# Frikallo/parakeet.cpp

Measured on NVIDIA H100. Metric: audio-seconds/sec (RTFx) tdt-ctc-110m 10s clips, higher is better.
Workload: dtype bf16x3

## Files before the change

parakeet.cpp_b200/csrc/engine.cu:

```cuda
#include "engine.h"

#include <algorithm>
#include <cstdlib>
#include <unordered_map>

namespace pk_detail {
std::string &create_err() {
    thread_local std::string s;
    return s;
}
}
#define g_create_err (create_err())


pk_status pk_engine::get_vec(const SafeTensors &st, const std::string &name, int n, float **out) {
    std::vector<float> h;
    std::string e;
    if (!st.read_f32(name, h, n, e)) return fail(PK_ERR_MISSING, e);
    *out = upload(h);
    return *out ? PK_OK : fail(PK_ERR_CUDA, "cudaMalloc failed for " + name);
}

pk_status pk_engine::finish_weight(std::vector<float> &w, std::vector<float> *b, int N, int K, GemmWeight &out) {
    out.N = N;
// ... 312 lines not shown
    logmel = dalloc<float>(B * (size_t)Fmax * c.mel_bins);
    mel_part = dalloc<float>(mel_part_floats((int)B, c.mel_bins));
    feats = dalloc<float>(B * (size_t)Fmax * c.mel_bins);
    sub1 = act_alloc(rows2, C);
    sub2 = dalloc<float>(rows2 * C);
    sub3 = act_alloc(rows3, C);
    sub4 = act_alloc(rows3, C);
    if (cfg.math != PK_MATH_FP32 && sub4.hi && (!make_tc_operand(&sub4.tc, sub4.hi, sub4.lo, Mx, (size_t)C * f3n, 128) || !make_tc_operand(&sub4.tc32, sub4.hi, sub4.lo, Mx, (size_t)C * f3n, 32))) sub4.hi = nullptr;
    x = dalloc<float>(Mx * d);
    ln = act_alloc(Mx, d);
    ffh = act_alloc(Mx, c.ff);
    qkv = dalloc<float>(Mx * 3 * d);
    if (cfg.math != PK_MATH_FP32 && (c.d_model / c.n_heads == 64 || c.d_model / c.n_heads == 128)) {
        qkvp_hi = dalloc<bf16>(Mx * 2 * d);
        qkvp_lo = dalloc<bf16>(Mx * 2 * d);
        if (!qkvp_hi || !qkvp_lo) return fail(PK_ERR_CUDA, "cudaMalloc failed (qkv planes)");
    }
    ctx = act_alloc(Mx, d);
    glu = dalloc<float>(Mx * d);
    cv = act_alloc(Mx, d);
    const int ldv = (c.vocab + 3) & ~3;
    logits = dalloc<float>(Mx * ldv);
    EP = dalloc<float>(Mx * c.joint_hidden);
    best = dalloc<int32_t>(Mx);
    bconf = dalloc<float>(Mx);
    tok = dalloc<int32_t>(B * (1 + (size_t)cap));
    t_start = dalloc<int32_t>(B * (size_t)cap);
    t_end = dalloc<int32_t>(B * (size_t)cap);
    t_conf = dalloc<float>(B * (size_t)cap);
    Bpad = ((Bmax + 31) / 32) * 32;
    const size_t HS = (size_t)c.pred_hidden * Bpad;
    hbuf = dalloc<float>(HS * 2 * c.lstm_layers);
    zbuf = dalloc<float>((size_t)c.joint_hidden * Bpad);
    tdt_ints = dalloc<int32_t>((size_t)Bpad + 512);
    tdt_keys = dalloc<unsigned long long>((size_t)6 * Bpad + 8);
    const size_t PG = (size_t)3 * num_sms * Bpad;
    pl_max = dalloc<float>(PG);
    pl_sum = dalloc<float>(PG);
    skinny_ws_floats = (size_t)2 << 20;
    skinny_ws = dalloc<float>(skinny_ws_floats);
    skinny_tickets = dalloc<unsigned int>(SKINNY_TICKETS);
    if (skinny_tickets) cudaMemsetAsync(skinny_tickets, 0, SKINNY_TICKETS * sizeof(unsigned int), stream);
    if (!pl_sum || !tdt_keys || !hbuf || !x || !sub2 || !d_pcm || !t_conf || !skinny_ws || !skinny_tickets || !mel_part) return fail(PK_ERR_CUDA, "cudaMalloc failed (workspace)");
    if (cfg.math != PK_MATH_FP32 && (!sub1.hi || !sub3.hi || !sub4.hi || !ln.hi || !ffh.hi || !ctx.hi || !cv.hi))
        return fail(PK_ERR_CUDA, "workspace: cudaMalloc or cuTensorMapEncodeTiled failed for an activation operand");
    if (diar) {
        const int Dt = sf.t_hidden;
        t_x = dalloc<float>(Mx * Dt);
        t_qkv = dalloc<float>(Mx * 3 * Dt);
        if (cfg.math != PK_MATH_FP32) {
            t_kv_hi = dalloc<bf16>(Mx * 2 * Dt);
            if (cfg.math == PK_MATH_BF16X3) t_kv_lo = dalloc<bf16>(Mx * 2 * Dt);
            if (!t_kv_hi || (cfg.math == PK_MATH_BF16X3 && !t_kv_lo)) return fail(PK_ERR_CUDA, "cudaMalloc failed (k | v planes)");
        }
        probs = dalloc<float>(Mx * sf.max_speakers);
        t_ln = act_alloc(Mx, Dt);
        t_ctx = act_alloc(Mx, Dt);
        t_ff = act_alloc(Mx, sf.t_ff);
        if (!t_x || !t_qkv || !probs || (cfg.math == PK_MATH_FP32 ? (!t_ln.f32 || !t_ctx.f32 || !t_ff.f32) : (!t_ln.hi || !t_ctx.hi || !t_ff.hi)))
            return fail(PK_ERR_CUDA, "cudaMalloc or cuTensorMapEncodeTiled failed (transformer workspace)");
        PK_CUDA(cudaMallocHost(&h_probs, Mx * sf.max_speakers * sizeof(float)));
    }
    PK_CUDA(cudaMallocHost(&h_pcm, (B * (size_t)c.max_samples + 8) * sizeof(float)));
    PK_CUDA(cudaMallocHost(&h_meta, (size_t)(8 * (B + 1)) * sizeof(int32_t)));
    PK_CUDA(cudaMallocHost(&h_tok, B * (1 + (size_t)cap) * sizeof(int32_t)));
    PK_CUDA(cudaMallocHost(&h_ts, B * (size_t)cap * sizeof(int32_t)));
    PK_CUDA(cudaMallocHost(&h_te, B * (size_t)cap * sizeof(int32_t)));
    PK_CUDA(cudaMallocHost(&h_tc, B * (size_t)cap * sizeof(float)));
    return PK_OK;
}

pk_status pk_engine::set_batch_shapes(const int32_t *n_frames, const int64_t *offsets, int n) {
    if (n <= 0) return fail(PK_ERR_INVALID, "empty batch");
    if (n > Bmax) return fail(PK_ERR_CAPACITY, "batch of " + std::to_string(n) + " exceeds max_batch " + std::to_string(Bmax));
    n_utt = n;
    probs_valid = false;
// ... 274 lines not shown
                launch_ctc_boosted_decode(logprobs_dev, best, bconf, d_row_off, n_utt, c.vocab, c.vocab - 1, cap, boost_trie(), tok, t_start, t_end, t_conf, stream);
            else
                launch_ctc_collapse(best, bconf, d_row_off, n_utt, c.vocab - 1, cap, tok, t_start, t_end, t_conf, stream);
        }
    }
    launches += greedy ? 2 : 3;
    last_tdt = false;
    PK_CUDA(cudaGetLastError());
    return PK_OK;
}

pk_status pk_engine::run_tdt() {
    TdtParams p{};
    p.Bpad = ((n_utt + 31) / 32) * 32; p.n_utt = n_utt; p.max_sym = cfg.max_symbols;
    p.max_steps = maxT + cap + 2; p.row_off = d_row_off; p.hbuf = hbuf;
    p.boost_on = boosting() ? 1 : 0; p.trie = boost_trie(); p.boost_bits = boost_bits; p.trie_active = trie_active; p.trie_nact = trie_nact;
    return tdt_decode(p);
}

pk_status pk_engine::tdt_decode(TdtParams &p) {
    const pk_config &c = cfg;
    EpiParams ep;
    ep.kind = EPI_BIAS_F32;
    ep.out_f32 = EP;
    ep.ldo = c.joint_hidden;
    gemm(enc_operand(this), c.d_model, enc_proj, M, ep);

    p.P = c.pred_hidden; p.J = c.joint_hidden; p.V = c.vocab; p.D = c.n_durations; p.L = c.lstm_layers;
    p.cap = cap; p.n_dur = c.n_durations;
    for (int i = 0; i < 8; ++i) p.durations[i] = c.durations[i];
    p.EP = EP; p.G0 = G0;
    for (int l = 0; l < c.lstm_layers; ++l) { p.Whh[l] = Whh_s[l]; p.Wih[l] = Wih_s[l]; p.bih[l] = bih[l]; }
    p.Wp = Wp_s; p.Wout = Wout_s; p.bout = bout;
    p.z = zbuf;
    p.overflow = tdt_ints; p.bar = reinterpret_cast<unsigned int *>(tdt_ints + Bpad);
    p.pl_max = pl_max; p.pl_sum = pl_sum;
    p.key_lab = tdt_keys; p.key_dur = tdt_keys + 3 * (size_t)Bpad;
    p.dbg = reinterpret_cast<long long *>(tdt_keys + 6 * (size_t)Bpad);
    p.tok = tok; p.t_start = t_start; p.t_end = t_end; p.t_conf = t_conf;
    if (!p.carry) PK_CUDA(cudaMemsetAsync(p.hbuf, 0, (size_t)p.P * p.Bpad * 2 * p.L * sizeof(float), stream));
    cudaError_t ce;
    {
        Scope sc(this, CAT_TDT);
        ce = launch_tdt_decode(p, num_sms, stream);
    }
    launches += 2;
    last_tdt = true;
    if (ce != cudaSuccess) return fail(PK_ERR_CUDA, std::string("tdt_decode launch: ") + cudaGetErrorString(ce));
    PK_CUDA(cudaGetLastError());
    return PK_OK;
}

pk_status pk_engine::run_diar_head() {
    const int Dt = sf.t_hidden, H = sf.t_heads;
    const bool f32 = cfg.math == PK_MATH_FP32;
    Act xo;
    if (f32) xo.f32 = t_x; else xo = t_ln;
    ActBuf planes;
    if (!f32) planes = t_ln;
    {
        EpiParams ep;
        ep.kind = EPI_BIAS_F32;
        ep.out_f32 = t_x;
        ep.ldo = Dt;
        gemm(enc_operand(this), cfg.d_model, t_proj, M, ep);
        if (!f32) {
            Scope sc(this, CAT_LAYERNORM);
// ... 1503 lines not shown
```

parakeet.cpp_b200/csrc/engine.h:

```cpp
#pragma once
#include <cuda_runtime.h>

#include <algorithm>
#include <cmath>
#include <cstdio>
#include <cstring>
#include <functional>
#include <map>
#include <memory>
#include <string>
#include <tuple>
#include <vector>

#include "../../include/parakeet_b200.h"
#include "kernels.h"
#include "nccl_dl.h"
#include "safetensors.h"

using namespace pk;


namespace pk_detail {

std::string &create_err();
// ... 142 lines not shown
    int cap = 0;

    MelTables mel_tb{};
    float *c1_w, *c1_b, *dw1_w, *dw1_b, *dw2_w, *dw2_b;
    float *dw2_wt = nullptr;
    GemmWeight conv2, conv3, proj;
    std::vector<LayerW> layers;
    GemmWeight ctc_head;
    GemmWeight enc_proj;
    float *G0 = nullptr;
    float *Whh[PK_MAX_LSTM] = {}, *Wih[PK_MAX_LSTM] = {}, *bih[PK_MAX_LSTM] = {};
    float *Whh_um[PK_MAX_LSTM] = {}, *Wih_um[PK_MAX_LSTM] = {};
    float *Wp = nullptr, *Wout = nullptr, *bout = nullptr;
    bf16 *Whh_s[PK_MAX_LSTM] = {}, *Wih_s[PK_MAX_LSTM] = {}, *Wp_s = nullptr, *Wout_s = nullptr;

    float *d_pcm = nullptr;
    float *d_pcm_alt = nullptr;
    cudaEvent_t ev_pcm_free[2] = {}, ev_prefetch = nullptr;
    int pcm_cur = 0;
    cudaEvent_t ev_join = nullptr;
    struct { const float *pcm = nullptr; int32_t n = 0; std::vector<int64_t> off; bool valid = false; } pref;
    int64_t *d_pcm_off = nullptr;
    int32_t *d_frame_off = nullptr, *d_s2_off = nullptr, *d_row_off = nullptr, *d_t2_rows = nullptr;
    float *logmel = nullptr, *feats = nullptr;
    float *mel_part = nullptr;
    Act sub1, sub3, sub4, ln, ffh, ctx, cv;
    float *sub2 = nullptr, *x = nullptr, *qkv = nullptr, *glu = nullptr, *logits = nullptr, *EP = nullptr;
    bf16 *qkvp_hi = nullptr, *qkvp_lo = nullptr;
    int32_t *best = nullptr;
    float *bconf = nullptr;
    int32_t *tok = nullptr, *t_start = nullptr, *t_end = nullptr;
    float *t_conf = nullptr;
    int Bpad = 0;
    float *hbuf = nullptr, *cbuf = nullptr, *zbuf = nullptr, *pl_max = nullptr, *pl_sum = nullptr;
    int32_t *tdt_ints = nullptr;
    unsigned long long *tdt_keys = nullptr;
    float *h_pcm = nullptr;
    int32_t *h_meta = nullptr;
    int32_t *h_tok = nullptr, *h_ts = nullptr, *h_te = nullptr;
    float *h_tc = nullptr;

    struct GraphEntry { cudaGraphExec_t exec = nullptr; int64_t launches = 0; int seen = 0; };
    std::map<std::string, GraphEntry> graphs;
    bool use_graphs = true;
    bool attn_tc = true;

    int n_utt = 0;
    std::vector<int64_t> pcm_off;
    std::vector<int32_t> frame_off, s2_off, row_off, t2_rows;
    int maxF = 0, maxT2 = 0, maxT = 0, M = 0, M2 = 0;

    int32_t *job_tok = nullptr, *job_all = nullptr;
    int64_t job_cap_rows = 0, job_rows = 0, job_alloc_rows = 0;
    int job_world = 1;
    int32_t *h_job = nullptr;
    size_t h_job_ints = 0;
    float *job_pcm = nullptr;
    size_t job_pcm_cap = 0;
    std::vector<int64_t> job_off;
    const float *pcm_src = nullptr;
    float *d_raw = nullptr;
    size_t d_raw_cap = 0;
    int64_t *d_raw_off = nullptr;
    void *nccl_comm = nullptr;
    int nccl_rank = 0, nccl_world = 1;
    bool last_tdt = false;
    int32_t truncated = 0;
// ... 126 lines not shown
```

parakeet.cpp_b200/csrc/kernel_hooks.cu:

```cuda
#include <algorithm>
#include <cmath>
#include <cstring>
#include <vector>

#include "../../include/parakeet_b200.h"
#include "kernels.h"

using namespace pk;

namespace {

constexpr size_t kGuard = (size_t)64 << 10;

struct HookCtx {
    cudaStream_t st = nullptr;
    std::vector<void *> ptrs;
    struct Guarded {
        uint8_t *base;
        size_t bytes;
    };
    std::vector<Guarded> outs;
    bool ok = true;

    explicit HookCtx(int device) {
// ... 308 lines not shown
    auto split = [&](const float *w, int rows, int K) {
        float *dw = cx.upload(w, (size_t)rows * K);
        bf16 *s = static_cast<bf16 *>(cx.alloc((size_t)rows * 2 * K * sizeof(bf16)));
        if (s) launch_tdt_split_rows(dw, rows, K, s, cx.st);
        return static_cast<const bf16 *>(s);
    };
    std::vector<float> um((size_t)4 * P * P);
    for (int l = 0; l < L; ++l) {
        lstm_unit_major(in->W_hh[l], P, um.data());
        p.Whh[l] = split(um.data(), 4 * P, P);
        if (l > 0) {
            lstm_unit_major(in->W_ih[l], P, um.data());
            p.Wih[l] = split(um.data(), 4 * P, P);
            p.bih[l] = cx.upload(in->b_ih[l], (size_t)4 * P);
        }
    }
    p.Wp = split(in->W_p, J, P);
    p.Wout = split(in->W_out, NO, J);
    p.bout = cx.upload(in->b_out, NO);
    bf16 *hb = cx.guarded<bf16>(2 * L * 2 * HS);
    bf16 *zb = cx.guarded<bf16>((size_t)2 * Bpad * J);
    {
        std::vector<float> h((size_t)L * 2 * HS, 0.f);
        if (in->carry)
            for (int l = 0; l < L; ++l)
                for (int b = 0; b < n; ++b) memcpy(&h[(size_t)l * 2 * HS + (size_t)b * P], in->h0 + ((size_t)l * n + b) * P, (size_t)P * 4);
        float *dh = cx.upload(h.data(), h.size());
        if (!cx.ok) return PK_ERR_CUDA;
        ActBuf sh; sh.hi = hb; sh.lo = hb + (size_t)L * 2 * HS;
        launch_split(dh, h.size(), sh, cx.st);
    }
    p.hbuf = reinterpret_cast<float *>(hb);
    p.z = reinterpret_cast<float *>(zb);
    p.tok = cx.guarded<int32_t>((size_t)n * (1 + cap));
    p.t_start = cx.guarded<int32_t>((size_t)n * cap);
    p.t_end = cx.guarded<int32_t>((size_t)n * cap);
    p.t_conf = cx.guarded<float>((size_t)n * cap);
    p.overflow = cx.guarded<int32_t>(n);
    constexpr int kMaxGrid = 256;
    p.pl_max = static_cast<float *>(cx.alloc((size_t)3 * kMaxGrid * Bpad * sizeof(float)));
    p.pl_sum = static_cast<float *>(cx.alloc((size_t)3 * kMaxGrid * Bpad * sizeof(float)));
    p.key_lab = static_cast<unsigned long long *>(cx.alloc((size_t)3 * Bpad * 8));
    p.key_dur = static_cast<unsigned long long *>(cx.alloc((size_t)3 * Bpad * 8));
    p.bar = static_cast<unsigned int *>(cx.alloc(1024 * sizeof(unsigned int)));
    p.dbg = static_cast<long long *>(cx.alloc(8 * sizeof(long long)));
    if (in->carry) {
        p.carry = 1;
        std::vector<float> c((size_t)L * Bpad * P, 0.f);
        for (int l = 0; l < L; ++l)
            memcpy(&c[(size_t)l * Bpad * P], in->c0 + (size_t)l * n * P, (size_t)n * P * 4);
        p.c_state = cx.guarded<float>(c.size());
        p.tok_state = cx.guarded<int32_t>(n);
        p.frame_base = cx.upload(in->frame_base, n);
        if (!cx.ok || cudaMemcpy(p.c_state, c.data(), c.size() * 4, cudaMemcpyHostToDevice) != cudaSuccess ||
            cudaMemcpy(p.tok_state, in->tok0, (size_t)n * 4, cudaMemcpyHostToDevice) != cudaSuccess)
            return PK_ERR_CUDA;
    }
    const int BW = (V + 31) / 32;
    if (bin) {
        if (D == 0 || !bin->row_off || !bin->boost || (in->carry && (!bin->trie_active0 || !bin->trie_nact0))) return PK_ERR_INVALID;
        std::vector<int32_t> slots((size_t)n * BOOST_SLOT_INTS, 0), act((size_t)n * BOOST_MAX_ACTIVE, 0), nact(n, 1), first, tk, cd;
        std::vector<uint32_t> bits((size_t)n * BW, 0u);
        for (int b = 0; b < n; ++b) {
            int32_t *slot = &slots[(size_t)b * BOOST_SLOT_INTS], *tok = slot + BOOST_SLOT_NODES + 1, *child = tok + BOOST_SLOT_EDGES;
            if (bin->row_off[b + 1] < bin->row_off[b]) return PK_ERR_INVALID;
            if (bin->row_off[b + 1] > bin->row_off[b]) {
// ... 493 lines not shown
```

parakeet.cpp_b200/csrc/kernels.h:

```cpp
#pragma once
#include <cuda.h>

#include <functional>
#include <string>
#include <vector>

#include "pk_common.cuh"

#define PK_MAX_LSTM 4

struct pk_lm;
struct pk_vocab;

namespace pk {

struct MelTables {
    const float *window;
    const float2 *tw256;
    const float2 *tw512;
    const float *fb_w;
    const int32_t *fb_start, *fb_len, *fb_off;
    int fb_nnz;
};
MelTables build_mel_tables(int n_mels, const std::function<void *(const void *, size_t)> &upload);
// ... 155 lines not shown
constexpr int CTC_BEAM_THREADS = 256;
void launch_ctc_frame_topk(const float *logprobs, int M, int V, int width, int32_t *topk_id, float *topk_lp, float *blank_lp,
                           cudaStream_t st);
std::string ctc_beam_tables(const pk_lm *lm, const pk_vocab *vocab, int V, const std::function<void *(const void *, size_t)> &upload,
                            DeviceLM *lm_out, DevicePieces *pc_out);
uint64_t ctc_beam_tables_id(const pk_lm *lm, const pk_vocab *vocab, int V);
void launch_ctc_beam(const float *logprobs, const int32_t *topk_id, const float *topk_lp, const float *blank_lp,
                     const int32_t *row_off, int n_utt, int V, int width, int cap, const DeviceLM &lm, const DevicePieces &pieces,
                     int32_t *bp, int32_t *tok, int32_t *t_start, int32_t *t_end, float *t_conf, cudaStream_t st);

constexpr int CTC_ALIGN_THREADS = 256;
size_t ctc_align_smem_bytes();
void launch_ctc_align(const float *logprobs, const int32_t *row_off, int n_utt, int V, const int32_t *tgt, const int32_t *tgt_off,
                      uint8_t *bp, int bp_stride, int32_t *best, float *conf, double *score, double *loglik, int32_t *path,
                      cudaStream_t st);

struct TdtParams {
    int P, J, V, D, L, Bpad, n_utt, cap, max_steps, n_dur;
    int max_sym;
    int out_in_smem, wih_in_smem, smem_lstm_floats;
    int wstage_rows;
    int durations[8];
    const float *EP;
    const int32_t *row_off;
    const float *G0;
    const bf16 *Whh[PK_MAX_LSTM];
    const bf16 *Wih[PK_MAX_LSTM];
    const float *bih[PK_MAX_LSTM];
    const bf16 *Wp;
    const bf16 *Wout;
    const float *bout;
    float *hbuf;
    float *z;
    int32_t *overflow;
    float *pl_max, *pl_sum;
    unsigned long long *key_lab, *key_dur;
    unsigned int *bar;
    long long *dbg;
    int32_t *tok;
    int32_t *t_start, *t_end;
    float *t_conf;
    int carry;
    float *c_state;
    int32_t *tok_state;
    const int32_t *frame_base;
    int boost_on;
    DeviceTrie trie;
    uint32_t *boost_bits;
    int32_t *trie_active, *trie_nact;
};
struct TdtLaunchCtl {
    int cluster = 0;
    bool no_stage = false;
    int grid = 0, CL = 0, UPC = 0, OPC = 0;
    int out_in_smem = 0, wih_in_smem = 0, staged_ih = 0, wstage_rows = 0;
};
cudaError_t launch_tdt_decode(TdtParams p, int num_sms, cudaStream_t st, TdtLaunchCtl *ctl = nullptr);
void lstm_unit_major(const float *src, int P, float *dst);
void tdt_pass_profile(long long *out8, bool reset);
void launch_tdt_split_rows(const float *src, int rows, int K, bf16 *dst, cudaStream_t st);

}
```

parakeet.cpp_b200/csrc/tdt.cu:

```cuda
#include <cstring>
#include <map>

#include "kernels.h"

namespace pk {
namespace {

constexpr int NWARP = 8;
constexpr int NTHR = NWARP * 32;
constexpr int BCH = 64;
constexpr int RG = 80;
constexpr int RLD = BCH + 4;
constexpr int MYMAX = 40;
constexpr int NPV = MYMAX * BCH / NTHR;

__device__ __forceinline__ uint32_t smem_addr(const void *p) { return (uint32_t)__cvta_generic_to_shared(p); }
__device__ __forceinline__ void cp_async16(uint32_t dst, const void *gsrc) {
    asm volatile("cp.async.cg.shared.global [%0], [%1], 16;" ::"r"(dst), "l"(gsrc) : "memory");
}
__device__ __forceinline__ void cp_async8(uint32_t dst, const void *gsrc) {
    asm volatile("cp.async.ca.shared.global [%0], [%1], 8;" ::"r"(dst), "l"(gsrc) : "memory");
}
__device__ __forceinline__ void cp_async_commit_wait_all() {
    asm volatile("cp.async.commit_group;" ::: "memory");
    asm volatile("cp.async.wait_group 0;" ::: "memory");
}
__device__ __forceinline__ void mma_bf16(float (&d)[4], const uint32_t (&a)[4], uint32_t b0, uint32_t b1) {
    asm volatile(
        "mma.sync.aligned.m16n8k16.row.col.f32.bf16.bf16.f32 {%0, %1, %2, %3}, {%4, %5, %6, %7}, {%8, %9}, {%0, %1, %2, %3};"
        : "+f"(d[0]), "+f"(d[1]), "+f"(d[2]), "+f"(d[3])
        : "r"(a[0]), "r"(a[1]), "r"(a[2]), "r"(a[3]), "r"(b0), "r"(b1));
}
__device__ __forceinline__ void ldsm_x4(uint32_t (&r)[4], uint32_t addr) {
    asm volatile("ldmatrix.sync.aligned.m8n8.x4.shared.b16 {%0, %1, %2, %3}, [%4];"
                 : "=r"(r[0]), "=r"(r[1]), "=r"(r[2]), "=r"(r[3]) : "r"(addr));
}
template <bool WS>
__device__ __forceinline__ uint32_t ldw32(const bf16 *p) {
    uint32_t v;
    if (WS) asm("ld.shared.b32 %0, [%1];" : "=r"(v) : "r"(smem_addr(p)));
    else asm("ld.global.nc.b32 %0, [%1];" : "=r"(v) : "l"(p));
    return v;
}
__device__ __forceinline__ void store_split(bf16 *hi, bf16 *lo, size_t idx, float v) {
    const bf16 h = __float2bfloat16_rn(v);
    hi[idx] = h;
    lo[idx] = __float2bfloat16_rn(v - __bfloat162float(h));
// ... 125 lines not shown
    if (prof) pt2 = clock64();
    store_partials<NBH>(acc, red);
    cluster_sync_all();
    if (prof) pt3 = clock64();
    uint32_t peer[CL];
#pragma unroll
    for (int q = 0; q < CL; ++q) peer[q] = mapa_rank(smem_addr(red), (uint32_t)q);
#pragma unroll
    for (int j = 0; j < NPV; ++j) {
        const int idx = threadIdx.x + j * NTHR, i = idx / BCH, b2 = idx % BCH;
        if (i < nmy && bc + b2 < Bpad) {
            const int r = myrow(i);
            const uint32_t off = (uint32_t)(r * RLD + b2) * 4u;
            float s = 0.f;
#pragma unroll
            for (int q = 0; q < CL; ++q) s += ld_cluster_f32(peer[q] + off);
            fin(i, r, bc + b2, s, pv[j]);
        }
    }
    __syncthreads();
    if (prof) {
        const long long pt4 = clock64();
        g_pass_clk[0] += pt1 - pt0;
        g_pass_clk[1] += pt2 - pt1;
        g_pass_clk[2] += pt3 - pt2;
        g_pass_clk[3] += pt4 - pt3;
        g_pass_clk[4] += 1;
    }
}

struct NoPost {
    __device__ __forceinline__ void operator()() const {}
};
template <int CL, bool WS1, bool WS2, typename X1, typename X2, typename MyRow, typename Pre, typename Fin, typename Post = NoPost>
__device__ __forceinline__ void cluster_pass_n(const bf16 *W1, int RS1, int LO1, X1 x1, const bf16 *W2, int RS2, int LO2, X2 x2,
                                               size_t lo_off, int R, int KS, int Bpad, int bc, bf16 *xs, float *red, int nmy,
                                               MyRow myrow, Pre pre, Fin fin, Post post = Post(), bool stage_x1 = true) {
    if (R <= 16) cluster_pass<CL, 1, WS1, WS2>(W1, RS1, LO1, x1, W2, RS2, LO2, x2, lo_off, R, KS, Bpad, bc, xs, red, nmy, myrow, pre, fin, post, stage_x1);
    else if (R <= 32) cluster_pass<CL, 2, WS1, WS2>(W1, RS1, LO1, x1, W2, RS2, LO2, x2, lo_off, R, KS, Bpad, bc, xs, red, nmy, myrow, pre, fin, post, stage_x1);
    else if (R <= 48) cluster_pass<CL, 3, WS1, WS2>(W1, RS1, LO1, x1, W2, RS2, LO2, x2, lo_off, R, KS, Bpad, bc, xs, red, nmy, myrow, pre, fin, post, stage_x1);
    else cluster_pass<CL, 5, WS1, WS2>(W1, RS1, LO1, x1, W2, RS2, LO2, x2, lo_off, R, KS, Bpad, bc, xs, red, nmy, myrow, pre, fin, post, stage_x1);
}

constexpr int GBAR = 8, GBAR_STRIDE = 32;
__device__ __forceinline__ void grid_arrive(unsigned int *counter) {
    __syncthreads();
    if (threadIdx.x == 0) {
        __threadfence();
        atomicAdd(counter + (blockIdx.x % GBAR) * GBAR_STRIDE, 1u);
    }
}
__device__ __forceinline__ void grid_wait(unsigned int *counter, unsigned int round ) {
    if (threadIdx.x < 32) {
        const int l = threadIdx.x;
        if (l < GBAR) {
            const unsigned int members = (gridDim.x - l + GBAR - 1) / GBAR;
            const unsigned int target = members * round;
            unsigned int v, spin = 0;
            do {
                asm volatile("ld.acquire.gpu.global.u32 %0, [%1];" : "=r"(v) : "l"(counter + l * GBAR_STRIDE) : "memory");
                if (++spin > (1u << 28)) __trap();
            } while (v < target);
        }
        __syncwarp();
        if (threadIdx.x == 0) __threadfence();
    }
    __syncthreads();
}

__device__ __forceinline__ unsigned long long pack_key(float v, int idx) {
    unsigned int u = __float_as_uint(v);
    u = (u & 0x80000000u) ? ~u : (u | 0x80000000u);
    return ((unsigned long long)u << 32) | (unsigned long long)(0xFFFFFFFFu - (unsigned int)idx);
}
// ... 32 lines not shown
__device__ __forceinline__ void boost_row_reset(const DeviceTrie &trie, int V, int b, uint32_t *bits, int32_t *active, int32_t *nact) {
    active[(size_t)b * BOOST_MAX_ACTIVE] = 0;
    nact[b] = 1;
    boost_mark_bits(trie_row(trie, b), active + (size_t)b * BOOST_MAX_ACTIVE, 1, V, bits + (size_t)b * ((V + 31) >> 5));
}

__device__ __noinline__ float boost_advance(const DeviceTrie &trie, int b, int token, float key, int V, uint32_t *boost_bits,
                                            int32_t *trie_active, int32_t *trie_nact) {
    const TrieRow tr = trie_row(trie, b);
    if (tr.empty()) return key;
    uint32_t *bits = boost_bits + (size_t)b * ((V + 31) >> 5);
    const float raw = ((bits[token >> 5] >> (token & 31)) & 1u) ? key - tr.boost : key;
    int32_t *act = trie_active + (size_t)b * BOOST_MAX_ACTIVE;
    const int na = trie_nact[b];
    int32_t nxt[BOOST_MAX_ACTIVE];
    int nn = 1;
    nxt[0] = 0;
    for (int a = 0; a < na; ++a) {
        const int node = act[a];
        for (int e = tr.first[node]; e < tr.first[node + 1]; ++e)
            if (tr.tok[e] == token) {
                const int ch = tr.child[e];
                bool dup = false;
                for (int q = 0; q < nn; ++q) dup |= nxt[q] == ch;
                if (!dup && nn < BOOST_MAX_ACTIVE) nxt[nn++] = ch;
            }
    }
    for (int q = 0; q < nn; ++q) act[q] = nxt[q];
    trie_nact[b] = nn;
    boost_mark_bits(tr, act, nn, V, bits);
    return raw;
}

template <int CL, bool BOOST>
__global__ void __launch_bounds__(NTHR, 1) tdt_decode_kernel(TdtParams p) {
    extern __shared__ __align__(16) float sm[];
    const int G = gridDim.x, g = blockIdx.x, tid = threadIdx.x;
    const int NC = G / CL;
    const int cid = (int)cluster_id_x(), rank = (int)cluster_ctarank();
    const int P = p.P, J = p.J, V = p.V, D = p.D, L = p.L, Bpad = p.Bpad;
    const int NO = V + D;
    const TdtGeom ge = tdt_geom(P, J, NO, NC, CL);
    const int u0 = min(cid * ge.UPC, P), u1 = min(u0 + ge.UPC, P), nU = u1 - u0;
    const int j0 = min(cid * ge.JPC, J), j1 = min(j0 + ge.JPC, J);
    const int o0 = min(cid * ge.OPC, NO), o1 = min(o0 + ge.OPC, NO);
    const int KSP = ge.KSP, KSJ = ge.KSJ;
    const int kP0 = rank * KSP, kJ0 = rank * KSJ;
    const int RSP = 2 * (KSP + 4), RSJ = 2 * (KSJ + 4);

    float *red = sm;
    float *gsm = red + RG * RLD;
    bf16 *xs = reinterpret_cast<bf16 *>(gsm + MYMAX * BCH);
    const int KSmax = max(KSP, KSJ);
    float *csm = reinterpret_cast<float *>(xs + (size_t)2 * min(BCH, Bpad) * (KSmax + 8));
    int *s_cur = reinterpret_cast<int *>(csm + (size_t)L * 2 * ge.MU * Bpad);
    int *s_token = s_cur + Bpad, *s_tpos = s_token + Bpad, *s_active = s_tpos + Bpad, *s_ntok = s_active + Bpad;
    int *s_pend = s_ntok + Bpad;
    float *s_vraw = reinterpret_cast<float *>(s_pend + Bpad);
    const bool rnnt = p.n_dur == 0;
    int *s_nsym = reinterpret_cast<int *>(s_vraw + Bpad);
    bf16 *wbf = reinterpret_cast<bf16 *>(s_nsym + (rnnt ? Bpad : 0));
    auto stage_rows = [&](bf16 *dst, const bf16 *src, int rows, int K, int k0, int KS) {
        const int RS = 2 * (KS + 4), n8 = KS / 4;
        for (int i = tid; i < rows * n8; i += blockDim.x) {
            const int r = i / n8, pc = i - r * n8;
            const uint2 *s = reinterpret_cast<const uint2 *>(src + (size_t)r * 2 * K + k0) + pc;
            uint2 *d = reinterpret_cast<uint2 *>(dst + (size_t)r * RS) + pc;
            *d = *s;
            *reinterpret_cast<uint2 *>(reinterpret_cast<bf16 *>(d) + KS + 4) = *reinterpret_cast<const uint2 *>(reinterpret_cast<const bf16 *>(s) + K);
        }
    };
    const bf16 *w_hh[PK_MAX_LSTM], *w_ih[PK_MAX_LSTM];
    {
// ... 67 lines not shown
    const size_t HS = (size_t)P * Bpad;
    bf16 *hb = reinterpret_cast<bf16 *>(p.hbuf), *zb = reinterpret_cast<bf16 *>(p.z);
    const size_t h_lo = (size_t)L * 2 * HS, z_lo = (size_t)J * Bpad;
    const size_t KB = (size_t)Bpad;
    const size_t PB = (size_t)G * Bpad;
    unsigned int nbar = 0;
    auto finalize_conf = [&](int buf) {
        const int warp = tid >> 5, lane = tid & 31;
        for (int b = g + warp * G; b < p.n_utt; b += G * NWARP) {
            const int slot = s_pend[b];
            if (slot < 0) continue;
            constexpr int QMAX = 8;
            float m[QMAX], sv[QMAX];
#pragma unroll
            for (int i = 0; i < QMAX; ++i) {
                const int q = lane + 32 * i;
                m[i] = q < G ? p.pl_max[buf * PB + (size_t)q * Bpad + b] : -INFINITY;
                sv[i] = q < G ? p.pl_sum[buf * PB + (size_t)q * Bpad + b] : 0.f;
            }
            float gmax = -INFINITY;
#pragma unroll
            for (int i = 0; i < QMAX; ++i) gmax = fmaxf(gmax, m[i]);
            gmax = warp_max(gmax);
            float s = 0.f;
#pragma unroll
            for (int i = 0; i < QMAX; ++i)
                if (m[i] > -INFINITY) s += sv[i] * expf(m[i] - gmax);
            s = warp_sum(s);
            if (lane == 0)
                p.t_conf[(size_t)b * p.cap + slot] = (BOOST && !trie_row(p.trie, b).empty()) ? expf(s_vraw[b] - gmax) / s : 1.0f / s;
        }
    };
    auto nox = [&](int) { return static_cast<const bf16 *>(nullptr); };

    long long tacc[8] = {0, 0, 0, 0, 0, 0, 0, 0}, tprev = clock64();
    auto tick = [&](int slot) {
        const long long now = clock64();
        tacc[slot] += now - tprev;
        tprev = now;
    };
    int step = 0;
    for (;; ++step) {
        const int kb = step % 3;
        if (g == 0)
            for (int b = tid; b < Bpad; b += blockDim.x) {
                p.key_lab[((step + 1) % 3) * KB + b] = 0ull;
                p.key_dur[((step + 1) % 3) * KB + b] = 0ull;
            }
        const bool staged_ih = !p.wih_in_smem && L > 1 && p.wstage_rows >= nU * 4 && nU <= RG / 4 && KSP == KSJ;
        if (staged_ih && L == 2) stage_rows_async(wstage, p.Wih[1] + (size_t)u0 * 4 * 2 * P, nU * 4, P, kP0, KSP);
        for (int l = 0; l < L; ++l) {
            if (staged_ih && L > 2 && l >= 1) stage_rows_async(wstage, p.Wih[l] + (size_t)u0 * 4 * 2 * P, nU * 4, P, kP0, KSP);
            for (int bc = 0; bc < Bpad; bc += BCH)
                for (int ug = 0; ug < nU; ug += RG / 4) {
                    const int nu = min(RG / 4, nU - ug), R = nu * 4;
                    const int myu = (nu - rank + CL - 1) / CL;
                    auto myrow = [&](int i) { return ((rank + CL * (i >> 2)) << 2) | (i & 3); };
                    auto pre_g = [&](int r, int b) {
                        const int u = u0 + ug + (r >> 2), gt = r & 3;
                        return (l == 0) ? p.G0[(size_t)s_token[b] * 4 * P + gt * P + u] : p.bih[l][gt * P + u];
                    };
                    auto fin_g = [&](int i, int, int b, float v, float e) { gsm[i * BCH + (b - bc)] = v + e; };
                    auto xprev = [&](int b) { return hb + ((size_t)(l * 2 + s_cur[b])) * HS + (size_t)b * P + kP0; };
                    const bf16 *W1 = w_hh[l] + (size_t)ug * 4 * RSP;
                    if (l == 0) {
                        cluster_pass_n<CL, true, true>(W1, RSP, KSP + 4, xprev, nullptr, 0, 0, nox, h_lo, R, KSP, Bpad, bc, xs, red,
                                                       myu * 4, myrow, pre_g, fin_g);
                    } else {
                        auto xh = [&](int b) { return hb + ((size_t)((l - 1) * 2 + (1 - s_cur[b]))) * HS + (size_t)b * P + kP0; };
                        if (p.wih_in_smem)
                            cluster_pass_n<CL, true, true>(W1, RSP, KSP + 4, xprev, w_ih[l] + (size_t)ug * 4 * RSP, RSP, KSP + 4, xh, h_lo, R,
                                                           KSP, Bpad, bc, xs, red, myu * 4, myrow, pre_g, fin_g);
                        else if (staged_ih)
                            cluster_pass_n<CL, true, true>(W1, RSP, KSP + 4, xprev, wstage, RSP, KSP + 4, xh, h_lo, R,
                                                           KSP, Bpad, bc, xs, red, myu * 4, myrow, pre_g, fin_g);
                        else
                            cluster_pass_n<CL, true, false>(W1, RSP, KSP + 4, xprev, w_ih[l] + (size_t)ug * 4 * 2 * P, 2 * P, P, xh, h_lo, R,
                                                            KSP, Bpad, bc, xs, red, myu * 4, myrow, pre_g, fin_g);
                    }
                    for (int idx = tid; idx < myu * BCH; idx += blockDim.x) {
                        const int mi = idx / BCH, bb = idx % BCH, b = bc + bb;
                        if (b >= Bpad) continue;
                        const int u = u0 + ug + rank + CL * mi;
                        const int cslot = ug / CL + mi;
                        const float gi = gsm[(mi * 4 + 0) * BCH + bb], gf = gsm[(mi * 4 + 1) * BCH + bb];
                        const float gg = gsm[(mi * 4 + 2) * BCH + bb], go = gsm[(mi * 4 + 3) * BCH + bb];
                        const int cu = s_cur[b];
                        const float c_old = csm[((size_t)(l * 2 + cu) * ge.MU + cslot) * Bpad + b];
                        const float c_new = sigmoidf_(gf) * c_old + sigmoidf_(gi) * tanhf(gg);
                        const float h_new = sigmoidf_(go) * tanhf(c_new);
                        csm[((size_t)(l * 2 + 1 - cu) * ge.MU + cslot) * Bpad + b] = c_new;
                        store_split(hb, hb + h_lo, ((size_t)(l * 2 + 1 - cu)) * HS + (size_t)b * P + u, h_new);
                    }
                    if (ug + RG / 4 < nU || bc + BCH < Bpad) cluster_sync_all();
                }
            tick(0);
            grid_arrive(p.bar);
            if (l == L - 1) {
                if (step > 0) finalize_conf((step - 1) % 3);
                __syncthreads();
                for (int b = tid; b < Bpad; b += blockDim.x) s_pend[b] = -1;
            }
            grid_wait(p.bar, ++nbar);
            tick(1);
        }
        for (int bc = 0; bc < Bpad; bc += BCH)
            for (int rg = j0; rg < j1; rg += RG) {
                const int R = min(RG, j1 - rg);
                const int nmy = (R - rank + CL - 1) / CL;
                cluster_pass_n<CL, true, true>(
                    w_p + (size_t)(rg - j0) * RSP, RSP, KSP + 4,
                    [&](int b) { return hb + ((size_t)((L - 1) * 2 + (1 - s_cur[b]))) * HS + (size_t)b * P + kP0; }, nullptr, 0, 0, nox,
                    h_lo, R, KSP, Bpad, bc, xs, red, nmy, [&](int i) { return rank + CL * i; },
                    [&](int r, int b) {
                        if (b >= p.n_utt) return 0.f;
                        const int T = p.row_off[b + 1] - p.row_off[b];
                        if (T <= 0) return 0.f;
                        const int t = min(s_tpos[b], T - 1);
                        return p.EP[(size_t)(p.row_off[b] + t) * J + rg + r];
                    },
                    [&](int, int r, int b, float v, float e) { store_split(zb, zb + z_lo, (size_t)b * J + rg + r, fmaxf(v + e, 0.f)); });
                if (rg + RG < j1 || bc + BCH < Bpad) cluster_sync_all();
            }
        tick(2);
        grid_arrive(p.bar);
        grid_wait(p.bar, ++nbar);
        tick(3);
        const bool staged_out = !p.out_in_smem && p.wstage_rows >= 16;
        const int RGo = staged_out ? p.wstage_rows : RG;
        for (int bc = 0; bc < Bpad; bc += BCH) {
            float lmax = -INFINITY, lsum = 0.f, dmax = -INFINITY;
            int lidx = 0x7fffffff, didx = 0x7fffffff;
            float kmax = -INFINITY;
            int kidx = 0x7fffffff;
            const int BW = (V + 31) >> 5;
            if (staged_out && o1 > o0) stage_rows_async(wstage, p.Wout + (size_t)o0 * 2 * J, min(RGo, o1 - o0), J, kJ0, KSJ);
            for (int rg = o0; rg < o1; rg += RGo) {
                const int R = min(RGo, o1 - rg);
                const int nmy = (R - rank + CL - 1) / CL;
                auto xz = [&](int b) { return zb + (size_t)b * J + kJ0; };
                auto myrow = [&](int i) { return rank + CL * i; };
                auto pb = [&](int r, int) { return p.bout[rg + r]; };
                auto fl = [&](int i, int, int b, float v, float e) { gsm[i * BCH + (b - bc)] = v + e; };
                const bool first_pass = rg == o0;
                if (p.out_in_smem) {
                    cluster_pass_n<CL, true, true>(w_o + (size_t)(rg - o0) * RSO, RSO, LOO, xz, nullptr, 0, 0, nox, z_lo, R, KSJ, Bpad, bc, xs,
                                                   red, nmy, myrow, pb, fl, NoPost(), first_pass);
                } else if (staged_out) {
                    auto next_tile = [&]() {
                        const int rn = rg + RGo;
                        __syncthreads();
                        if (rn < o1) stage_rows_async(wstage, p.Wout + (size_t)rn * 2 * J, min(RGo, o1 - rn), J, kJ0, KSJ);
                    };
                    cluster_pass_n<CL, true, true>(wstage, RSJ, KSJ + 4, xz, nullptr, 0, 0, nox, z_lo, R, KSJ, Bpad, bc, xs, red, nmy, myrow, pb, fl,
                                                   next_tile, first_pass);
// ... 66 lines not shown
                if (n < p.cap && (b % G) == g) {
                    int32_t *row = p.tok + (size_t)b * (1 + p.cap);
                    row[1 + n] = lidx;
                    const int base = p.carry ? p.frame_base[b] : 0;
                    p.t_start[(size_t)b * p.cap + n] = base + t;
                    p.t_end[(size_t)b * p.cap + n] = p.carry ? base + t + max(skip, 1) - 1 : min(t + max(skip, 1) - 1, T - 1);
                    row[0] = n + 1;
                }
                if (n < p.cap) s_pend[b] = n;
                if (BOOST && (b % G) == g) {
                    s_vraw[b] = boost_advance(p.trie, b, lidx, lmax, V, p.boost_bits, p.trie_active, p.trie_nact);
                }
                s_ntok[b] = n + 1;
                s_token[b] = lidx;
                s_cur[b] = 1 - s_cur[b];
                t += skip;
                if (rnnt && ++s_nsym[b] >= p.max_sym) {
                    t += 1;
                    s_nsym[b] = 0;
                }
                if (n + 1 >= p.cap) {
                    act = false;
                    if ((b % G) == g) p.overflow[b] = 1;
                }
            }
            s_tpos[b] = t;
            if (t >= T) act = false;
            s_active[b] = act ? 1 : 0;
            any |= act ? 1 : 0;
        }
        any = __syncthreads_or(any);
        tick(6);
        if (!any || step + 1 >= p.max_steps) break;
    }
    if (p.dbg && g == 0 && tid == 0) {
        for (int i = 0; i < 7; ++i) p.dbg[i] = tacc[i];
        p.dbg[7] = step + 1;
    }
    finalize_conf(step % 3);
    if (p.carry) {
        for (int l = 0; l < L; ++l)
            for_my_units([&](int u, int cslot) {
                for (int b = tid; b < Bpad; b += blockDim.x) {
                    const int cu = s_cur[b];
                    p.c_state[((size_t)l * Bpad + b) * P + u] = csm[((size_t)(l * 2 + cu) * ge.MU + cslot) * Bpad + b];
                    if (cu == 1) {
                        const size_t src = ((size_t)(l * 2 + 1)) * HS + (size_t)b * P + u, dst = ((size_t)(l * 2 + 0)) * HS + (size_t)b * P + u;
                        hb[dst] = hb[src];
                        hb[h_lo + dst] = hb[h_lo + src];
                    }
                }
            });
        for (int b = g + tid * G; b < p.n_utt; b += G * blockDim.x) p.tok_state[b] = s_token[b];
    }
    cluster_sync_all();
}

__global__ void tdt_init_kernel(TdtParams p) {
    const int b = blockIdx.x * blockDim.x + threadIdx.x;
    if (b < GBAR * GBAR_STRIDE) p.bar[b] = 0u;
    if (b < 3 * p.Bpad) {
        p.key_lab[b] = 0ull;
        p.key_dur[b] = 0ull;
    }
    if (b < p.n_utt) {
        p.tok[(size_t)b * (1 + p.cap)] = 0;
// ... 21 lines not shown

size_t tdt_smem_bytes(const TdtParams &p, int n_clusters, int CL, bool *out_in_smem, bool *wih_in_smem, int *lstm_floats, int *wstage_rows) {
    const TdtGeom ge = tdt_geom(p.P, p.J, p.V + p.D, n_clusters, CL);
    const size_t budget = 225 * 1024 / sizeof(float);
    const int KSmax = ge.KSP > ge.KSJ ? ge.KSP : ge.KSJ;
    const int xrows = p.Bpad < BCH ? p.Bpad : BCH;
    size_t fixed = (size_t)RG * RLD + (size_t)MYMAX * BCH + (size_t)2 * xrows * (KSmax + 8) / 2 + (size_t)p.L * 2 * ge.MU * p.Bpad +
                   (p.n_dur == 0 ? 8 : 7) * (size_t)p.Bpad;
    const size_t hh = (size_t)p.L * ge.UPC * 4 * (ge.KSP + 4), ih = (size_t)(p.L - 1) * ge.UPC * 4 * (ge.KSP + 4);
    const size_t wp = (size_t)ge.JPC * (ge.KSP + 4), wo = (size_t)ge.OPC * (ge.KSJ + 4);
    size_t total = fixed + hh + wp;
    *wih_in_smem = (ih == 0) || (total + ih <= budget);
    *lstm_floats = (int)(hh + (*wih_in_smem ? ih : 0));
    *out_in_smem = total + (*wih_in_smem ? ih : 0) + wo <= budget;
    *wstage_rows = 0;
    if (*out_in_smem) {
        total += (*wih_in_smem ? ih : 0) + wo;
    } else {
        const size_t left = budget > total ? budget - total : 0;
        int rows = (int)(left / (size_t)(ge.KSJ + 4));
        rows = rows >= 80 ? 80 : (rows >= 64 ? 64 : (rows >= 48 ? 48 : (rows >= 32 ? 32 : (rows >= 16 ? 16 : 0))));
        *wstage_rows = rows;
        total += (size_t)rows * (ge.KSJ + 4);
        *wih_in_smem = (ih == 0) || (total + ih <= budget);
        *lstm_floats = (int)(hh + (*wih_in_smem ? ih : 0));
        if (*wih_in_smem) total += ih;
    }
    return total * sizeof(float);
}

template <int CL>
cudaError_t launch_cl(TdtParams p, int num_sms, cudaStream_t st, bool *fits, TdtLaunchCtl *ctl) {
    *fits = false;
    const auto kernel = p.boost_on ? tdt_decode_kernel<CL, true> : tdt_decode_kernel<CL, false>;
    if (p.P % (16 * CL) || p.J % (16 * CL)) return cudaSuccess;
    int nc = num_sms / CL;
    if (nc * CL > 256) nc = 256 / CL;
    cudaLaunchConfig_t cfg = {};
    cudaLaunchAttribute attr[2];
    attr[0].id = cudaLaunchAttributeClusterDimension;
    attr[0].val.clusterDim.x = CL;
    attr[0].val.clusterDim.y = 1;
    attr[0].val.clusterDim.z = 1;
    attr[1].id = cudaLaunchAttributeCooperative;
    attr[1].val.cooperative = 1;
    cfg.blockDim = dim3(NTHR);
    cfg.stream = st;
    cfg.attrs = attr;
    cfg.numAttrs = 2;
    cudaError_t err;
    for (int iter = 0; iter < 2; ++iter) {
        bool out_in_smem, wih_in_smem;
        int lstm_floats, wstage_rows;
        const size_t smem = tdt_smem_bytes(p, nc, CL, &out_in_smem, &wih_in_smem, &lstm_floats, &wstage_rows);
        if (smem > 227 * 1024) return cudaSuccess;
        err = cudaFuncSetAttribute(kernel, cudaFuncAttributeMaxDynamicSharedMemorySize, (int)smem);
        if (err != cudaSuccess) { cudaGetLastError(); return cudaSuccess; }
        cfg.gridDim = dim3(nc * CL);
        cfg.dynamicSmemBytes = smem;
        int max_clusters = 0;
        err = cudaOccupancyMaxActiveClusters(&max_clusters, kernel, &cfg);
        if (err != cudaSuccess) { cudaGetLastError(); return cudaSuccess; }
        if (max_clusters >= nc) {
            p.out_in_smem = out_in_smem ? 1 : 0;
            p.wih_in_smem = wih_in_smem ? 1 : 0;
            p.smem_lstm_floats = lstm_floats;
            p.wstage_rows = (ctl && ctl->no_stage) ? 0 : wstage_rows;
// ... 90 lines not shown
```

Before: 43960.

## Fuse LSTM hidden-gate matvec into joint projection pass for single-layer predictor

For single-layer LSTM predictors, the recurrent Whh·h product for the next step is folded into the same cluster pass that computes the joint predictor projection, writing gate pre-activations to a new global buffer. The cell update then runs at the end of each step, combining those stored gates with the token embedding gates, so the separate LSTM phase and its grid barrier are skipped after the first step. This aims to cut one grid-wide synchronisation and one weight-streaming pass per decode step, in exchange for larger row groups (RG2 at cluster size 4), an extra global buffer and a more complex per-step schedule.

```diff
diff --git a/parakeet.cpp_b200/csrc/engine.cu b/parakeet.cpp_b200/csrc/engine.cu
--- a/parakeet.cpp_b200/csrc/engine.cu
+++ b/parakeet.cpp_b200/csrc/engine.cu
@@ -368,6 +368,7 @@
     const size_t HS = (size_t)c.pred_hidden * Bpad;
     hbuf = dalloc<float>(HS * 2 * c.lstm_layers);
     zbuf = dalloc<float>((size_t)c.joint_hidden * Bpad);
+    if (c.lstm_layers == 1) ghbuf = dalloc<float>(HS * 4);
     tdt_ints = dalloc<int32_t>((size_t)Bpad + 512);
     tdt_keys = dalloc<unsigned long long>((size_t)6 * Bpad + 8);
     const size_t PG = (size_t)3 * num_sms * Bpad;
@@ -377,7 +378,7 @@
     skinny_ws = dalloc<float>(skinny_ws_floats);
     skinny_tickets = dalloc<unsigned int>(SKINNY_TICKETS);
     if (skinny_tickets) cudaMemsetAsync(skinny_tickets, 0, SKINNY_TICKETS * sizeof(unsigned int), stream);
-    if (!pl_sum || !tdt_keys || !hbuf || !x || !sub2 || !d_pcm || !t_conf || !skinny_ws || !skinny_tickets || !mel_part) return fail(PK_ERR_CUDA, "cudaMalloc failed (workspace)");
+    if (!pl_sum || !tdt_keys || !hbuf || (c.lstm_layers == 1 && !ghbuf) || !x || !sub2 || !d_pcm || !t_conf || !skinny_ws || !skinny_tickets || !mel_part) return fail(PK_ERR_CUDA, "cudaMalloc failed (workspace)");
     if (cfg.math != PK_MATH_FP32 && (!sub1.hi || !sub3.hi || !sub4.hi || !ln.hi || !ffh.hi || !ctx.hi || !cv.hi))
         return fail(PK_ERR_CUDA, "workspace: cudaMalloc or cuTensorMapEncodeTiled failed for an activation operand");
     if (diar) {
@@ -718,7 +719,7 @@
     p.EP = EP; p.G0 = G0;
     for (int l = 0; l < c.lstm_layers; ++l) { p.Whh[l] = Whh_s[l]; p.Wih[l] = Wih_s[l]; p.bih[l] = bih[l]; }
     p.Wp = Wp_s; p.Wout = Wout_s; p.bout = bout;
-    p.z = zbuf;
+    p.z = zbuf; p.gh = ghbuf;
     p.overflow = tdt_ints; p.bar = reinterpret_cast<unsigned int *>(tdt_ints + Bpad);
     p.pl_max = pl_max; p.pl_sum = pl_sum;
     p.key_lab = tdt_keys; p.key_dur = tdt_keys + 3 * (size_t)Bpad;
diff --git a/parakeet.cpp_b200/csrc/engine.h b/parakeet.cpp_b200/csrc/engine.h
--- a/parakeet.cpp_b200/csrc/engine.h
+++ b/parakeet.cpp_b200/csrc/engine.h
@@ -198,7 +198,7 @@
     int32_t *tok = nullptr, *t_start = nullptr, *t_end = nullptr;
     float *t_conf = nullptr;
     int Bpad = 0;
-    float *hbuf = nullptr, *cbuf = nullptr, *zbuf = nullptr, *pl_max = nullptr, *pl_sum = nullptr;
+    float *hbuf = nullptr, *ghbuf = nullptr, *zbuf = nullptr, *pl_max = nullptr, *pl_sum = nullptr;
     int32_t *tdt_ints = nullptr;
     unsigned long long *tdt_keys = nullptr;
     float *h_pcm = nullptr;
diff --git a/parakeet.cpp_b200/csrc/kernel_hooks.cu b/parakeet.cpp_b200/csrc/kernel_hooks.cu
--- a/parakeet.cpp_b200/csrc/kernel_hooks.cu
+++ b/parakeet.cpp_b200/csrc/kernel_hooks.cu
@@ -364,6 +364,7 @@
     }
     p.hbuf = reinterpret_cast<float *>(hb);
     p.z = reinterpret_cast<float *>(zb);
+    p.gh = static_cast<float *>(cx.alloc((size_t)Bpad * 4 * P * sizeof(float)));
     p.tok = cx.guarded<int32_t>((size_t)n * (1 + cap));
     p.t_start = cx.guarded<int32_t>((size_t)n * cap);
     p.t_end = cx.guarded<int32_t>((size_t)n * cap);
diff --git a/parakeet.cpp_b200/csrc/kernels.h b/parakeet.cpp_b200/csrc/kernels.h
--- a/parakeet.cpp_b200/csrc/kernels.h
+++ b/parakeet.cpp_b200/csrc/kernels.h
@@ -211,6 +211,7 @@
     const float *bout;
     float *hbuf;
     float *z;
+    float *gh;
     int32_t *overflow;
     float *pl_max, *pl_sum;
     unsigned long long *key_lab, *key_dur;
diff --git a/parakeet.cpp_b200/csrc/tdt.cu b/parakeet.cpp_b200/csrc/tdt.cu
--- a/parakeet.cpp_b200/csrc/tdt.cu
+++ b/parakeet.cpp_b200/csrc/tdt.cu
@@ -13,6 +13,8 @@
 constexpr int RLD = BCH + 4;
 constexpr int MYMAX = 40;
 constexpr int NPV = MYMAX * BCH / NTHR;
+constexpr int RG2 = 112;
+static_assert(RG2 * RLD <= RG * RLD + MYMAX * BCH && RG2 <= MYMAX * 4, "RG2 rows fit the two buffers and MYMAX per CTA at CL = 4");
 
 __device__ __forceinline__ uint32_t smem_addr(const void *p) { return (uint32_t)__cvta_generic_to_shared(p); }
 __device__ __forceinline__ void cp_async16(uint32_t dst, const void *gsrc) {
@@ -204,14 +206,15 @@
 struct NoPost {
     __device__ __forceinline__ void operator()() const {}
 };
-template <int CL, bool WS1, bool WS2, typename X1, typename X2, typename MyRow, typename Pre, typename Fin, typename Post = NoPost>
+template <int CL, bool WS1, bool WS2, int NBMAX = RG / 16, typename X1, typename X2, typename MyRow, typename Pre, typename Fin, typename Post = NoPost>
 __device__ __forceinline__ void cluster_pass_n(const bf16 *W1, int RS1, int LO1, X1 x1, const bf16 *W2, int RS2, int LO2, X2 x2,
                                                size_t lo_off, int R, int KS, int Bpad, int bc, bf16 *xs, float *red, int nmy,
                                                MyRow myrow, Pre pre, Fin fin, Post post = Post(), bool stage_x1 = true) {
     if (R <= 16) cluster_pass<CL, 1, WS1, WS2>(W1, RS1, LO1, x1, W2, RS2, LO2, x2, lo_off, R, KS, Bpad, bc, xs, red, nmy, myrow, pre, fin, post, stage_x1);
     else if (R <= 32) cluster_pass<CL, 2, WS1, WS2>(W1, RS1, LO1, x1, W2, RS2, LO2, x2, lo_off, R, KS, Bpad, bc, xs, red, nmy, myrow, pre, fin, post, stage_x1);
     else if (R <= 48) cluster_pass<CL, 3, WS1, WS2>(W1, RS1, LO1, x1, W2, RS2, LO2, x2, lo_off, R, KS, Bpad, bc, xs, red, nmy, myrow, pre, fin, post, stage_x1);
-    else cluster_pass<CL, 5, WS1, WS2>(W1, RS1, LO1, x1, W2, RS2, LO2, x2, lo_off, R, KS, Bpad, bc, xs, red, nmy, myrow, pre, fin, post, stage_x1);
+    else if (R <= RG || NBMAX == RG / 16) cluster_pass<CL, 5, WS1, WS2>(W1, RS1, LO1, x1, W2, RS2, LO2, x2, lo_off, R, KS, Bpad, bc, xs, red, nmy, myrow, pre, fin, post, stage_x1);
+    else cluster_pass<CL, NBMAX, WS1, WS2>(W1, RS1, LO1, x1, W2, RS2, LO2, x2, lo_off, R, KS, Bpad, bc, xs, red, nmy, myrow, pre, fin, post, stage_x1);
 }
 
 constexpr int GBAR = 8, GBAR_STRIDE = 32;
@@ -310,13 +313,13 @@
     return raw;
 }
 
-template <int CL, bool BOOST>
+template <int CL, bool BOOST, bool FUSED>
 __global__ void __launch_bounds__(NTHR, 1) tdt_decode_kernel(TdtParams p) {
     extern __shared__ __align__(16) float sm[];
     const int G = gridDim.x, g = blockIdx.x, tid = threadIdx.x;
     const int NC = G / CL;
     const int cid = (int)cluster_id_x(), rank = (int)cluster_ctarank();
-    const int P = p.P, J = p.J, V = p.V, D = p.D, L = p.L, Bpad = p.Bpad;
+    const int P = p.P, J = p.J, V = p.V, D = p.D, L = FUSED ? 1 : p.L, Bpad = p.Bpad;
     const int NO = V + D;
     const TdtGeom ge = tdt_geom(P, J, NO, NC, CL);
     const int u0 = min(cid * ge.UPC, P), u1 = min(u0 + ge.UPC, P), nU = u1 - u0;
@@ -450,6 +453,14 @@
         }
     };
     auto nox = [&](int) { return static_cast<const bf16 *>(nullptr); };
+    auto cell_update = [&](int l, int u, int cslot, int b, float gi, float gf, float gg, float go) {
+        const int cu = s_cur[b];
+        const float c_old = csm[((size_t)(l * 2 + cu) * ge.MU + cslot) * Bpad + b];
+        const float c_new = sigmoidf_(gf) * c_old + sigmoidf_(gi) * tanhf(gg);
+        const float h_new = sigmoidf_(go) * tanhf(c_new);
+        csm[((size_t)(l * 2 + 1 - cu) * ge.MU + cslot) * Bpad + b] = c_new;
+        store_split(hb, hb + h_lo, ((size_t)(l * 2 + 1 - cu)) * HS + (size_t)b * P + u, h_new);
+    };
 
     long long tacc[8] = {0, 0, 0, 0, 0, 0, 0, 0}, tprev = clock64();
     auto tick = [&](int slot) {
@@ -457,6 +468,8 @@
         tacc[slot] += now - tprev;
         tprev = now;
     };
+    constexpr bool fused = FUSED;
+    constexpr int RGF = fused && CL == 4 ? RG2 : RG;
     int step = 0;
     for (;; ++step) {
         const int kb = step % 3;
@@ -467,7 +480,7 @@
             }
         const bool staged_ih = !p.wih_in_smem && L > 1 && p.wstage_rows >= nU * 4 && nU <= RG / 4 && KSP == KSJ;
         if (staged_ih && L == 2) stage_rows_async(wstage, p.Wih[1] + (size_t)u0 * 4 * 2 * P, nU * 4, P, kP0, KSP);
-        for (int l = 0; l < L; ++l) {
+        for (int l = 0; l < (fused && step > 0 ? 0 : L); ++l) {
             if (staged_ih && L > 2 && l >= 1) stage_rows_async(wstage, p.Wih[l] + (size_t)u0 * 4 * 2 * P, nU * 4, P, kP0, KSP);
             for (int bc = 0; bc < Bpad; bc += BCH)
                 for (int ug = 0; ug < nU; ug += RG / 4) {
@@ -501,14 +514,8 @@
                         if (b >= Bpad) continue;
                         const int u = u0 + ug + rank + CL * mi;
                         const int cslot = ug / CL + mi;
-                        const float gi = gsm[(mi * 4 + 0) * BCH + bb], gf = gsm[(mi * 4 + 1) * BCH + bb];
-                        const float gg = gsm[(mi * 4 + 2) * BCH + bb], go = gsm[(mi * 4 + 3) * BCH + bb];
-                        const int cu = s_cur[b];
-                        const float c_old = csm[((size_t)(l * 2 + cu) * ge.MU + cslot) * Bpad + b];
-                        const float c_new = sigmoidf_(gf) * c_old + sigmoidf_(gi) * tanhf(gg);
-                        const float h_new = sigmoidf_(go) * tanhf(c_new);
-                        csm[((size_t)(l * 2 + 1 - cu) * ge.MU + cslot) * Bpad + b] = c_new;
-                        store_split(hb, hb + h_lo, ((size_t)(l * 2 + 1 - cu)) * HS + (size_t)b * P + u, h_new);
+                        cell_update(l, u, cslot, b, gsm[(mi * 4 + 0) * BCH + bb], gsm[(mi * 4 + 1) * BCH + bb], gsm[(mi * 4 + 2) * BCH + bb],
+                                    gsm[(mi * 4 + 3) * BCH + bb]);
                     }
                     if (ug + RG / 4 < nU || bc + BCH < Bpad) cluster_sync_all();
                 }
@@ -522,23 +529,30 @@
             grid_wait(p.bar, ++nbar);
             tick(1);
         }
+        const int rh = fused ? 4 * ge.UPC : 0, NR = rh + (j1 - j0);
         for (int bc = 0; bc < Bpad; bc += BCH)
-            for (int rg = j0; rg < j1; rg += RG) {
-                const int R = min(RG, j1 - rg);
+            for (int rg = 0; rg < NR; rg += RGF) {
+                const int R = min(RGF, NR - rg);
                 const int nmy = (R - rank + CL - 1) / CL;
-                cluster_pass_n<CL, true, true>(
-                    w_p + (size_t)(rg - j0) * RSP, RSP, KSP + 4,
+                cluster_pass_n<CL, true, true, RGF / 16>(
+                    (fused ? w_hh[0] : w_p) + (size_t)rg * RSP, RSP, KSP + 4,
                     [&](int b) { return hb + ((size_t)((L - 1) * 2 + (1 - s_cur[b]))) * HS + (size_t)b * P + kP0; }, nullptr, 0, 0, nox,
                     h_lo, R, KSP, Bpad, bc, xs, red, nmy, [&](int i) { return rank + CL * i; },
                     [&](int r, int b) {
-                        if (b >= p.n_utt) return 0.f;
+                        const int jr = rg + r - rh;
+                        if ((fused && jr < 0) || b >= p.n_utt) return 0.f;
                         const int T = p.row_off[b + 1] - p.row_off[b];
                         if (T <= 0) return 0.f;
                         const int t = min(s_tpos[b], T - 1);
-                        return p.EP[(size_t)(p.row_off[b] + t) * J + rg + r];
+                        return p.EP[(size_t)(p.row_off[b] + t) * J + j0 + jr];
                     },
-                    [&](int, int r, int b, float v, float e) { store_split(zb, zb + z_lo, (size_t)b * J + rg + r, fmaxf(v + e, 0.f)); });
-                if (rg + RG < j1 || bc + BCH < Bpad) cluster_sync_all();
+                    [&](int, int r, int b, float v, float e) {
+                        const int jr = rg + r - rh;
+                        if (!fused || jr >= 0) store_split(zb, zb + z_lo, (size_t)b * J + j0 + jr, fmaxf(v + e, 0.f));
+                        else if (rg + r < 4 * nU) p.gh[((size_t)b * P + u0) * 4 + rg + r] = v;
+                    },
+                    NoPost(), !fused || rg == 0);
+                if (rg + RGF < NR || bc + BCH < Bpad) cluster_sync_all();
             }
         tick(2);
         grid_arrive(p.bar);
@@ -671,6 +685,25 @@
         any = __syncthreads_or(any);
         tick(6);
         if (!any || step + 1 >= p.max_steps) break;
+        if (fused) {
+            constexpr int UPP = RG / 4 / CL;
+            for (int idx = tid; idx < ge.MU * p.n_utt; idx += blockDim.x) {
+                const int cslot = idx / p.n_utt, b = idx - cslot * p.n_utt;
+                const int ul = (cslot / UPP) * (RG / 4) + rank + CL * (cslot % UPP);
+                if (ul >= nU || s_pend[b] < 0) continue;
+                const int u = u0 + ul;
+                const float4 gh = *reinterpret_cast<const float4 *>(p.gh + ((size_t)b * P + u) * 4);
+                const float *g0 = p.G0 + (size_t)s_token[b] * 4 * P + u;
+                cell_update(0, u, cslot, b, gh.x + g0[0], gh.y + g0[P], gh.z + g0[2 * P], gh.w + g0[3 * P]);
+            }
+            tick(0);
+            grid_arrive(p.bar);
+            finalize_conf(kb);
+            __syncthreads();
+            for (int b = tid; b < Bpad; b += blockDim.x) s_pend[b] = -1;
+            grid_wait(p.bar, ++nbar);
+            tick(1);
+        }
     }
     if (p.dbg && g == 0 && tid == 0) {
         for (int i = 0; i < 7; ++i) p.dbg[i] = tacc[i];
@@ -758,7 +791,8 @@
 template <int CL>
 cudaError_t launch_cl(TdtParams p, int num_sms, cudaStream_t st, bool *fits, TdtLaunchCtl *ctl) {
     *fits = false;
-    const auto kernel = p.boost_on ? tdt_decode_kernel<CL, true> : tdt_decode_kernel<CL, false>;
+    const auto kernel = p.L == 1 ? (p.boost_on ? tdt_decode_kernel<CL, true, true> : tdt_decode_kernel<CL, false, true>)
+                                 : (p.boost_on ? tdt_decode_kernel<CL, true, false> : tdt_decode_kernel<CL, false, false>);
     if (p.P % (16 * CL) || p.J % (16 * CL)) return cudaSuccess;
     int nc = num_sms / CL;
     if (nc * CL > 256) nc = 256 / CL;
```

New measurement: 45070, median of 6. 1.03x the previous value.
